# jrkerns/pylinac

Measured on NVIDIA H100. Metric: EPID frames/sec (1024x1024) through PicketFence.analyze(), higher is better.
Workload: dtype u16 pixels / int exact sums / f64 profiles

## Files before the change

pylinac_b200/csrc/peaks.cuh:

```cuda
#pragma once
#include "common.cuh"

namespace epid {

constexpr int PK_WALK = 64;
#ifndef EPID_PK_MAXBLK
#define EPID_PK_MAXBLK 512
#endif
constexpr int PK_MAXBLK = EPID_PK_MAXBLK;
constexpr int PK_RANK_MAX = 768;
constexpr int PK_COOP = 32;

struct PeakArgs {
    double hmin;
    int distance;
    double pmin;
    double wmin;
    double rel_height;
    int max_number;
    int sort_by_height;
};

struct PeakWork {
    int cap;
    int* idx;
    double* prom;
    int* lbase;
    int* rbase;
    double* width_height;
    double* lip;
    double* rip;
    int* flag;
    double* skey;
    int* sidx;
    int* s_small;
};

__device__ __forceinline__ bool key_less(double ka, int ia, double kb, int ib) { return ka < kb || (ka == kb && ia < ib); }

__device__ inline void block_bitonic_sort(double* key, int* idx, int m) {
    for (int k = 2; k <= m; k <<= 1) {
        for (int j = k >> 1; j > 0; j >>= 1) {
            for (int i = threadIdx.x; i < m; i += blockDim.x) {
                const int l = i ^ j;
                if (l > i) {
                    const bool up = (i & k) == 0;
                    const double ka = key[i], kb = key[l];
                    const int ia = idx[i], ib = idx[l];
                    const bool sw = up ? key_less(kb, ib, ka, ia) : key_less(ka, ia, kb, ib);
                    if (sw) {
                        key[i] = kb; key[l] = ka;
                        idx[i] = ib; idx[l] = ia;
                    }
                }
            }
            __syncthreads();
        }
    }
}

__device__ inline int compact_by_flag(PeakWork& w, int count, bool have_props) {
    const int tid = threadIdx.x, nt = blockDim.x, lane = tid & 31, wid = tid >> 5, nw = nt >> 5;
    __syncthreads();
    int out = 0;
    for (int base = 0; base < count; base += nt) {
        const int i = base + tid;
        const bool keep = i < count && w.flag[i] != 0;
        int idx = 0, lb = 0, rb = 0;
// ... 94 lines not shown
            bool waiting = false;
            for (int i = tid; i < count; i += nt) {
                int st = cur[i];
                if (st == 2) {
                    const int pi = w.idx[i], ri = rank[i];
                    bool has_kept = false, blocked = false;
                    for (int k = i - 1; k >= 0 && pi - w.idx[k] < a.distance; k--) {
                        const int sk = cur[k];
                        if (sk == 1) { has_kept = true; break; }
                        if (sk == 2 && rank[k] > ri) { blocked = true; break; }
                    }
                    if (!has_kept && !blocked) {
                        for (int k = i + 1; k < count && w.idx[k] - pi < a.distance; k++) {
                            const int sk = cur[k];
                            if (sk == 1) { has_kept = true; break; }
                            if (sk == 2 && rank[k] > ri) { blocked = true; break; }
                        }
                    }
                    st = has_kept ? 0 : (blocked ? 2 : 1);
                    waiting = waiting || st == 2;
                }
                nxt[i] = st;
            }
            const int more = __syncthreads_or(waiting ? 1 : 0);
            int* t = cur; cur = nxt; nxt = t;
            if (!more) break;
        }
        if (cur != w.flag) {
            for (int i = tid; i < count; i += nt) w.flag[i] = cur[i];
        }
        count = compact_by_flag(w, count, false);
    }

    __shared__ double s_bmax[PK_MAXBLK], s_bmin[PK_MAXBLK];
    __shared__ unsigned short s_bpos[PK_MAXBLK];
    const bool have_tab = n <= 32 * PK_MAXBLK;
    if (have_tab) {
        const int lane = tid & 31, wid = tid >> 5, nw = nt >> 5;
        const int nblk = (n + 31) >> 5;
        __syncthreads();
        for (int b = wid; b < nblk; b += nw) {
            const int k = (b << 5) + lane;
            const bool in = k < n;
            const double v = in ? x[k] : 0.0;
            double vmax = in ? v : -__longlong_as_double(0x7ff0000000000000LL);
            double vmin = in ? v : __longlong_as_double(0x7ff0000000000000LL);
#pragma unroll
            for (int o = 16; o > 0; o >>= 1) {
                vmax = fmax(vmax, __shfl_xor_sync(0xffffffffu, vmax, o));
                vmin = fmin(vmin, __shfl_xor_sync(0xffffffffu, vmin, o));
            }
            const unsigned eq = __ballot_sync(0xffffffffu, in && v == vmin);
            if (lane == 0) {
                s_bmax[b] = vmax;
                s_bmin[b] = vmin;
                s_bpos[b] = (unsigned short)((__ffs(eq) - 1) | ((31 - __clz(eq)) << 8));
            }
        }
        __syncthreads();
        for (int i = tid; i < count; i += nt) {
            const int p = w.idx[i];
            const double xp = x[p];
            const int pb_ = p >> 5;
            double lmin = xp;
            int lb = p;
            bool stop = false;
            for (int k = p; k >= (pb_ << 5); k--) {
                const double v = x[k];
                if (!stop) {
                    if (v > xp) stop = true;
                    else if (v < lmin) { lmin = v; lb = k; }
                }
            }
            for (int b = pb_ - 1; b >= 0 && !stop; b--) {
                if (s_bmax[b] > xp) {
                    for (int k = (b << 5) + 31; k >= (b << 5); k--) {
                        const double v = x[k];
                        if (!stop) {
                            if (v > xp) stop = true;
                            else if (v < lmin) { lmin = v; lb = k; }
                        }
                    }
                } else if (s_bmin[b] < lmin) {
                    lmin = s_bmin[b];
                    lb = (b << 5) + (s_bpos[b] >> 8);
                }
            }
            double rmin = xp;
            int rb = p;
            stop = false;
            const int own_end = min(n - 1, (pb_ << 5) + 31);
            for (int k = p; k <= own_end; k++) {
// ... 187 lines not shown
```

pylinac_b200/csrc/pf_common.cuh:

```cuda
#pragma once
#include <cmath>

#include "filters.cuh"
#include "peaks.cuh"
#include "stats.cuh"

namespace epid {

constexpr int PF_P = EPID_PF_MAX_PICKETS;
constexpr int PF_L = EPID_PF_MAX_LEAVES;
constexpr int PROF_THREADS = 256;
constexpr int PROF_MAXN = STATS_MAX_DIM;
constexpr int PROF_PEAK_CAP = 512;
constexpr int WIN_WARPS = 4;
constexpr int WIN_CAP_PX = 4096;
constexpr int WIN_MAX_NC = 1024;
constexpr int WIN_MAX_NR = 64;
constexpr int FIN_THREADS = 256;

constexpr int PF_STATUS_DEFERRED = 90;

struct PfConst {
    epid_pf_params p;
    int H, W;
// ... 187 lines not shown
    const int wid = threadIdx.x >> 5, nw = blockDim.x >> 5, lane = threadIdx.x & 31;
    __syncthreads();
    if (n0 <= 1024 && n1 <= 1024) {
        for (int s = wid; s < 4; s += nw) {
            const bool second = s >= 2;
            const PctPlan& pp = (s & 1) ? (second ? p99_1 : p99_0) : (second ? p85_1 : p85_0);
            uint32_t va, vb;
            warp_select_pair_u32(second ? a1 : a0, second ? n1 : n0, pp.prev, pp.next, va, vb);
            if (lane == 0) { sel[2 * s] = va; sel[2 * s + 1] = vb; }
        }
    } else {
        for (int s = wid; s < 8; s += nw) {
            const bool second = s >= 4;
            const PctPlan& pp = (s & 2) ? (second ? p99_1 : p99_0) : (second ? p85_1 : p85_0);
            const int r = (s & 1) ? pp.next : pp.prev;
            const uint32_t v = warp_select_u32(second ? a1 : a0, second ? n1 : n0, r);
            if (lane == 0) sel[s] = v;
        }
    }
    __syncthreads();
    range0 = np_lerp((double)sel[2], (double)sel[3], p99_0.gamma) - np_lerp((double)sel[0], (double)sel[1], p85_0.gamma);
    range1 = np_lerp((double)sel[6], (double)sel[7], p99_1.gamma) - np_lerp((double)sel[4], (double)sel[5], p85_1.gamma);
    __syncthreads();
}

__host__ __device__ inline int pf_profile_len(int H, int W) { return ((H > W ? H : W) + 3) & ~3; }
__host__ __device__ inline size_t pf_profile_smem_bytes(int threads, int H, int W) {
    return sizeof(double) * (pf_profile_len(H, W) + 5 * PROF_PEAK_CAP) + sizeof(int) * (5 * PROF_PEAK_CAP + threads + 8) + 64 * sizeof(double);
}

__device__ inline void pf_profile_block(const PfConst& c, PfFrame& f, const uint32_t* __restrict__ rowsum,
                                        const uint32_t* __restrict__ colsum, const uint32_t* __restrict__ rowsum2,
                                        const uint32_t* __restrict__ colsum2, unsigned char* smraw, double d_colsum2 = 0.0,
                                        double d_rowsum2 = 0.0, int* counters = nullptr) {
    double* prof = reinterpret_cast<double*>(smraw);
    double* w_prom = prof + pf_profile_len(c.H, c.W);
    double* w_wh = w_prom + PROF_PEAK_CAP;
    double* w_lip = w_wh + PROF_PEAK_CAP;
    double* w_rip = w_lip + PROF_PEAK_CAP;
    double* w_skey = w_rip + PROF_PEAK_CAP;
    double* s_red = w_skey + PROF_PEAK_CAP;
    double* s_bcast = s_red + 32;
    int* w_idx = reinterpret_cast<int*>(s_bcast + 32);
    int* w_lb = w_idx + PROF_PEAK_CAP;
    int* w_rb = w_lb + PROF_PEAK_CAP;
    int* w_flag = w_rb + PROF_PEAK_CAP;
    int* w_sidx = w_flag + PROF_PEAK_CAP;
    int* w_small = w_sidx + PROF_PEAK_CAP;

    if (f.status != EPID_PF_OK) return;
    const int H = c.H, W = c.W;
    const int tid = threadIdx.x;
    const int NT = blockDim.x;
    const int NW = NT >> 5;

    int orient = c.p.orientation;
    if (orient < 0) {
        uint32_t* buf = reinterpret_cast<uint32_t*>(prof);
        double row_range, col_range;
        block_pct_ranges2(colsum2, W, c.p85[0], c.p99[0], rowsum2, H, c.p85[1], c.p99[1], buf, row_range, col_range);
        orient = (row_range < col_range) ? 1 : 0;
        if (counters && (d_colsum2 > 0.0 || d_rowsum2 > 0.0)) {
            const bool sure_lr = row_range + d_colsum2 + 1.0 < col_range - d_rowsum2;
            const bool sure_ud = row_range - d_colsum2 >= col_range + d_rowsum2 + 1.0;
            if (!sure_lr && !sure_ud) {
                if (threadIdx.x == 0) { atomicAdd(&counters[1], 1); f.status = PF_STATUS_DEFERRED; }
                return;
            }
        }
    }
    const int n = orient == 0 ? W : H;
    const int other = orient == 0 ? H : W;
    const uint32_t* raw = orient == 0 ? colsum : rowsum;
    const long long base = (long long)other * (long long)(f.inv ? f.mx : f.mn);
    double lmax = 0.0;
    for (int i = tid; i < n; i += NT) {
        const long long sg = f.inv ? base - (long long)raw[i] : (long long)raw[i] - base;
        const double v = (double)sg;
        prof[i] = v;
        lmax = fmax(lmax, v);
    }
    lmax = warp_max(lmax);
    if ((tid & 31) == 0) s_red[tid >> 5] = lmax;
    __syncthreads();
    if (tid == 0) {
        double m = 0.0;
        for (int i = 0; i < NW; i++) m = fmax(m, s_red[i]);
        s_bcast[0] = m;
    }
    __syncthreads();
    const double pmax = s_bcast[0];
    double lmin = 2.0;
    for (int i = tid; i < n; i += NT) {
        const double v = prof[i] / pmax;
        prof[i] = v;
        lmin = fmin(lmin, v);
    }
    lmin = warp_min(lmin);
    __syncthreads();
    if ((tid & 31) == 0) s_red[tid >> 5] = lmin;
    __syncthreads();
    if (tid == 0) {
        double m = 2.0;
        for (int i = 0; i < NW; i++) m = fmin(m, s_red[i]);
        s_bcast[1] = m;
    }
    __syncthreads();
    const double pmin = s_bcast[1];
    PeakArgs a;
    {
        const double val_range = 1.0 - pmin;
        double thr = c.p.height_threshold;
        if (thr >= 0.0 && thr <= 1.0) thr = pmin + thr * val_range;
        a.hmin = thr;
        a.distance = max((int)(0.02 * (double)n), 1);
        a.pmin = c.p.required_prominence;
        a.wmin = 0.0;
        a.rel_height = 1.0 - 0.5;
        a.max_number = c.p.num_pickets;
        a.sort_by_height = c.p.peak_sort == 1;
    }
    PeakWork w;
    w.cap = PROF_PEAK_CAP;
    w.idx = w_idx; w.prom = w_prom; w.lbase = w_lb; w.rbase = w_rb; w.width_height = w_wh; w.lip = w_lip; w.rip = w_rip;
    w.flag = w_flag; w.skey = w_skey; w.sidx = w_sidx; w.s_small = w_small;
    const int np = block_find_peaks(prof, n, a, w);
    if (tid == 0) {
        f.orientation = orient;
        if (np < 0 || np > PF_P) {
            f.status = EPID_PF_TOO_MANY_PICKETS;
        } else if (np == 0) {
            f.status = EPID_PF_NO_PICKETS;
        } else {
            f.n_pickets = np;
            int sorted[PF_P];
            for (int k = 0; k < np; k++) {
                const double lt = w.lip[k], rt = w.rip[k];
                const int idx = (int)rint(lt + (rt - lt) / 2.0);
                f.picket_idx[k] = idx;
                f.picket_val[k] = prof[idx];
                int j = k;
                while (j > 0 && sorted[j - 1] > idx) { sorted[j] = sorted[j - 1]; j--; }
                sorted[j] = idx;
            }
            double spacing = c.p.picket_spacing;
            if (spacing < 0) {
                const int nd = np - 1;
                if (nd <= 0) {
                    spacing = __longlong_as_double(0x7ff8000000000000LL);
                } else {
                    int d[PF_P];
                    for (int k = 0; k < nd; k++) {
                        const int v = sorted[k + 1] - sorted[k];
                        int j = k;
                        while (j > 0 && d[j - 1] > v) { d[j] = d[j - 1]; j--; }
                        d[j] = v;
                    }
                    spacing = (nd & 1) ? (double)d[nd / 2] : ((double)d[nd / 2 - 1] + (double)d[nd / 2]) / 2.0;
                }
            }
            f.spacing = spacing;
            if (spacing != spacing) f.status = EPID_PF_NAN_SPACING;
            const double n_axis = (double)(orient == 0 ? H : W);
            const double ratio = c.p.leaf_analysis_width_ratio;
            double pixel_range = n_axis / 2.0;
            pixel_range -= fmax(c.p.leaf_width_mm[0] * ratio, c.p.leaf_width_mm[c.p.n_leaves - 1] * ratio) * c.p.dpmm;
            int cnt = 0;
            for (int l = 0; l < c.p.n_leaves; l++)
                if (fabs(c.p.leaf_center_mm[l]) < pixel_range / c.p.dpmm) f.inview[cnt++] = (short)l;
            f.n_inview = cnt;
        }
    }
}

}
```

pylinac_b200/csrc/pf_stream.cu:

```cuda
#define EPID_PK_MAXBLK 2
#include "pf_common.cuh"
#include "tma.cuh"

namespace epid {

#ifndef EPID_ST_NCW
#define EPID_ST_NCW 12
#endif
constexpr int ST_NCW = EPID_ST_NCW;
constexpr int ST_THREADS = (ST_NCW + 1) * 32;
constexpr int ST_NST = 6;
constexpr int ST_KMAX = 8;
constexpr int ST_MAXROWS = 1024;
constexpr int PILOT_THREADS = 256;
constexpr int PILOT_BINS = 2048;
constexpr int PILOT_STEP = 32, PILOT_OFF = 16;
constexpr int TAIL_THREADS = 256;

struct PilotOut {
    uint32_t u_lo, a1, b1, l_hi;
};

struct ItemOut {
    uint32_t mn, mx;
    uint32_t cnt_a, cnt_b, cnt_lo, cnt_hi;
    uint32_t pad[2];
};

struct StreamGeom {
    int H, W;
    int K;
    int rows_per_item;
    int nvec;
    int nstrips;
    int wa;
    int row_bytes;
    int rps;
};

__device__ __forceinline__ void consumer_bar() { asm volatile("bar.sync 1, %0;" ::"n"(ST_NCW * 32) : "memory"); }
__device__ __forceinline__ uint4 lds128(uint32_t addr) {
    uint4 r;
    asm volatile("ld.shared.v4.u32 {%0,%1,%2,%3}, [%4];" : "=r"(r.x), "=r"(r.y), "=r"(r.z), "=r"(r.w) : "r"(addr));
    return r;
}

__device__ __forceinline__ int pilot_rows_of(int H) { return H > PILOT_OFF ? (H - PILOT_OFF + PILOT_STEP - 1) / PILOT_STEP : 0; }

__device__ __forceinline__ uint32_t pilot_scan_excl(uint32_t v, uint32_t* s_red, uint32_t* total) {
    const int lane = threadIdx.x & 31, wid = threadIdx.x >> 5;
    uint32_t inc = v;
#pragma unroll
    for (int o = 1; o < 32; o <<= 1) {
        const uint32_t t = __shfl_up_sync(0xffffffffu, inc, o);
        if (lane >= o) inc += t;
    }
    __syncthreads();
    if (lane == 31) s_red[wid] = inc;
    __syncthreads();
    if (wid == 0) {
        const uint32_t w = lane < PILOT_THREADS / 32 ? s_red[lane] : 0;
        uint32_t winc = w;
#pragma unroll
        for (int o = 1; o < 32; o <<= 1) {
            const uint32_t t = __shfl_up_sync(0xffffffffu, winc, o);
            if (lane >= o) winc += t;
        }
        if (lane < PILOT_THREADS / 32) s_red[lane] = winc - w;
        if (lane == 31) s_red[32] = winc;
    }
    __syncthreads();
    const uint32_t excl = s_red[wid] + inc - v;
    *total = s_red[32];
    return excl;
}

__device__ inline uint32_t pilot_find(const uint32_t* __restrict__ hist, uint32_t nb, uint32_t base, uint32_t rank, uint32_t* s_red,
                                      uint32_t* s_found) {
    const int tid = threadIdx.x;
    const uint32_t per = (nb + PILOT_THREADS - 1) / PILOT_THREADS;
    const uint32_t lo = min(nb, tid * per), hi = min(nb, lo + per);
    uint32_t c = 0;
    for (uint32_t i = lo; i < hi; i++) c += hist[i];
    uint32_t total;
    const uint32_t excl = pilot_scan_excl(c, s_red, &total);
    if (tid == 0) *s_found = rank < base ? 0xffffffffu : nb;
    __syncthreads();
    if (rank >= base) {
        const uint32_t k = rank - base;
        if (k >= excl && k < excl + c) {
            uint32_t acc = excl;
            for (uint32_t i = lo; i < hi; i++) {
                const uint32_t h = hist[i];
                if (k < acc + h) { *s_found = i; break; }
                acc += h;
            }
        }
    }
    __syncthreads();
    const uint32_t r = *s_found;
    __syncthreads();
    return r;
}

__global__ void __launch_bounds__(PILOT_THREADS)
k_pf_pilot(const StatsGeom g, const FrameRef* __restrict__ frames, int nframes, PilotOut* __restrict__ out) {
    __shared__ uint32_t hist[3][PILOT_BINS];
    __shared__ uint32_t bis_lo[4], bis_hi[4], bis_cnt[4], bis_rank[4];
    __shared__ uint32_t a0s[3], b0s[3], shs[3], below_s[3], eq_s[3];
    __shared__ uint32_t s_red[40], s_found, smin, smax;
    const int fi = blockIdx.x;
    if (fi >= nframes) return;
    const FrameRef frf = frames[fi];
    const int H = g.H, W = g.W;
    const int tid = threadIdx.x, lane = tid & 31, wid = tid >> 5;
    const uint32_t npix = (uint32_t)H * (uint32_t)W;
    const uint32_t k_lo[3] = {g.ranks[0], g.ranks[4], npix - 1 - g.ranks[3]};
    const uint32_t k_hi[3] = {g.ranks[1], g.ranks[5], npix - 1 - g.ranks[2]};
    for (int i = tid; i < 3 * PILOT_BINS; i += PILOT_THREADS) (&hist[0][0])[i] = 0;
    if (tid < 3) { below_s[tid] = 0; eq_s[tid] = 0; }
    if (tid == 0) { smin = 0xffffu; smax = 0; }
    uint32_t sv[8];
    {
        const int col = min(W - 1, (int)(((long long)tid * W) / PILOT_THREADS));
#pragma unroll
        for (int i = 0; i < 8; i++) {
            const int row = min(H - 1, (int)(((2 * i + 1) * (long long)H) / 16));
            sv[i] = __ldg(frf.origin + (size_t)row * frf.pitch + col);
        }
    }
    const uint32_t nT0 = PILOT_THREADS * 8;
    if (tid < 4) {
        const int b = tid == 0 ? 0 : (tid == 3 ? 2 : 1);
        const double fq = fmin((b == 1 ? 1.0 : 4.0) * (double)(tid == 1 ? k_lo[b] : k_hi[b]) / (double)npix, 0.999);
        const double sg = sqrt(fq * (1.0 - fq) * (double)nT0);
        const double ctr = fq * (double)nT0;
        double rr = (tid == 1) ? ctr - 5.0 * sg - 2.0 : ctr + 5.0 * sg + 3.0;
        rr = fmin(fmax(rr, 0.0), (double)(nT0 - 1));
        bis_rank[tid] = (uint32_t)rr;
        bis_lo[tid] = 0;
        bis_hi[tid] = 65535u;
        bis_cnt[tid] = 0;
    }
    __syncthreads();
    {
        uint32_t mnv = sv[0], mxv = sv[0];
#pragma unroll
        for (int i = 1; i < 8; i++) { mnv = min(mnv, sv[i]); mxv = max(mxv, sv[i]); }
        mnv = warp_min(mnv);
        mxv = warp_max(mxv);
        if (lane == 0) { atomicMin(&smin, mnv); atomicMax(&smax, mxv); }
    }
    for (int step = 0; step < 16; step++) {
        uint32_t cnt[4];
#pragma unroll
        for (int t = 0; t < 4; t++) {
            const uint32_t mid = (bis_lo[t] + bis_hi[t]) >> 1;
            uint32_t cc_ = 0;
#pragma unroll
            for (int i = 0; i < 8; i++) {
                const uint32_t v = t == 3 ? 65535u - sv[i] : sv[i];
                cc_ += v <= mid ? 1u : 0u;
            }
            cnt[t] = __reduce_add_sync(0xffffffffu, cc_);
        }
        if (lane < 4) atomicAdd(&bis_cnt[lane], lane == 0 ? cnt[0] : lane == 1 ? cnt[1] : lane == 2 ? cnt[2] : cnt[3]);
        __syncthreads();
        if (tid < 4) {
            const uint32_t mid = (bis_lo[tid] + bis_hi[tid]) >> 1;
            if (bis_cnt[tid] >= bis_rank[tid] + 1) bis_hi[tid] = mid; else bis_lo[tid] = mid + 1;
            bis_cnt[tid] = 0;
        }
        __syncthreads();
    }
    if (tid == 0) {
        uint32_t a[3], b[3];
        a[0] = smin;              b[0] = max(bis_lo[0], smin);
        a[1] = bis_lo[1];         b[1] = max(bis_lo[2], a[1]);
        a[2] = 65535u - smax;     b[2] = max(bis_lo[3], a[2]);
        for (int j = 0; j < 3; j++) {
            uint32_t sh = 0;
            while (((b[j] - a[j]) >> sh) >= (uint32_t)PILOT_BINS) sh++;
            a0s[j] = a[j];
            b0s[j] = b[j];
            shs[j] = sh;
        }
    }
    __syncthreads();
    const uint32_t a0[3] = {a0s[0], a0s[1], a0s[2]};
    const uint32_t wd[3] = {b0s[0] - a0s[0], b0s[1] - a0s[1], b0s[2] - a0s[2]};
    const uint32_t sh[3] = {shs[0], shs[1], shs[2]};
    uint32_t below[3] = {0, 0, 0}, eq[3] = {0, 0, 0};
    const int np_rows = pilot_rows_of(H);
    const bool aligned = true;
    const int mis = (int)((reinterpret_cast<uintptr_t>(frf.origin) >> 1) & 7);
    const int jf = (mis + 7) / 8, jl = (W + mis) / 8;
    const int cl = aligned ? min(W, max(0, jf * 8 - mis)) : 0;
    const int cr = aligned ? (jl > jf ? jl * 8 - mis : cl) : 0;
    auto put = [&](int j, uint32_t vv) {
        const int u = (int)vv - (int)a0[j];
        below[j] += (uint32_t)u >> 31;
        eq[j] += u == 0 ? 1u : 0u;
        if ((uint32_t)(u - 1) < wd[j]) atomicAdd(&hist[j][(uint32_t)u >> sh[j]], 1u);
    };
    for (int ri = wid; ri < np_rows; ri += PILOT_THREADS / 32) {
        const uint16_t* rowp = frf.origin + (size_t)(PILOT_OFF + PILOT_STEP * ri) * frf.pitch;
        for (int j = jf + lane; j < jl; j += 32) {
            const uint4 q = ldg_stream16(rowp - mis + j * 8);
            const uint32_t w[4] = {q.x, q.y, q.z, q.w};
            const uint32_t vm = __vminu2(__vminu2(w[0], w[1]), __vminu2(w[2], w[3]));
            const uint32_t vM = __vmaxu2(__vmaxu2(w[0], w[1]), __vmaxu2(w[2], w[3]));
            put(0, vm & 0xffffu);
            put(0, vm >> 16);
            put(2, 65535u - (vM & 0xffffu));
            put(2, 65535u - (vM >> 16));
#pragma unroll
            for (int t = 0; t < 4; t++) { put(1, w[t] & 0xffffu); put(1, w[t] >> 16); }
        }
    }
#pragma unroll
    for (int j = 0; j < 3; j++) {
        const uint32_t b = __reduce_add_sync(0xffffffffu, below[j]);
        const uint32_t e = __reduce_add_sync(0xffffffffu, eq[j]);
        if (lane == 0) { if (b) atomicAdd(&below_s[j], b); if (e) atomicAdd(&eq_s[j], e); }
    }
    __syncthreads();
    if (tid < 3 && eq_s[tid]) hist[tid][0] += eq_s[tid];
    __syncthreads();
    const uint32_t n_p = (uint32_t)np_rows * (uint32_t)(aligned ? cr - cl : W);
    uint32_t thr_lo[3], thr_hi[3];
    for (int j = 0; j < 3; j++) {
        const uint32_t nb = (wd[j] >> sh[j]) + 1;
        const double scale = (double)n_p / (double)npix;
        const double pop = j == 1 ? (double)n_p : (double)n_p / 4.0;
        const double fq = fmin((j == 1 ? 1.0 : 4.0) * ((double)k_lo[j] + 0.5) / (double)npix, 1.0);
        const double sg = sqrt(fq * (1.0 - fq) * pop);
        const double rl = (double)k_lo[j] * scale - 5.0 * sg - 2.0;
        const double ru = (double)k_hi[j] * scale + 5.0 * sg + 3.0;
        const uint32_t r_l = rl <= 0.0 ? 0u : (uint32_t)rl;
        const uint32_t r_u = (uint32_t)fmin(ru, fmax(pop - 1.0, 0.0));
        const uint32_t xa = pilot_find(hist[j], nb, below_s[j], r_l, s_red, &s_found);
        const uint32_t xb = pilot_find(hist[j], nb, below_s[j], r_u, s_red, &s_found);
        uint32_t lo_t = xa == 0xffffffffu ? a0[j] : a0[j] + (min(xa, nb - 1) << sh[j]);
        uint32_t hi_t = xb == 0xffffffffu ? a0[j] : a0[j] + (((min(xb, nb - 1) + 1) << sh[j]) - 1);
        hi_t = min(hi_t, 65535u);
        lo_t = min(lo_t, hi_t);
        thr_lo[j] = lo_t;
        thr_hi[j] = hi_t;
    }
    if (tid == 0) {
        PilotOut o;
        o.u_lo = thr_hi[0];
        o.a1 = thr_lo[1];
        o.b1 = thr_hi[1];
        o.l_hi = 65535u - thr_hi[2];
        out[fi] = o;
    }
}

struct StreamSh {
    unsigned long long full[ST_NST], empty[ST_NST];
    uint32_t mn, mx, cnt[4];
};

template <int VPL>
__global__ void __launch_bounds__(ST_THREADS, 1)
k_pf_stream(const StreamGeom sg, const FrameRef* __restrict__ frames, const PilotOut* __restrict__ pilot, int nitems,
            ItemOut* __restrict__ items, uint32_t* __restrict__ col_raw, uint32_t* __restrict__ col_cl,
            uint32_t* __restrict__ row_raw, uint32_t* __restrict__ row_cl) {
    extern __shared__ __align__(128) unsigned char smraw[];
    StreamSh* sh = reinterpret_cast<StreamSh*>(smraw);
    unsigned char* ring = smraw + 256;
    const int stage_bytes = sg.rps * sg.row_bytes;
    uint32_t* flush = reinterpret_cast<uint32_t*>(ring + (size_t)ST_NST * stage_bytes);
    const int tid = threadIdx.x, lane = tid & 31, wid = tid >> 5;
    if (tid == 0) {
        for (int s = 0; s < ST_NST; s++) { mbar_init(smem_u32(&sh->full[s]), 1); mbar_init(smem_u32(&sh->empty[s]), ST_NCW); }
// ... 155 lines not shown
          const uint32_t* __restrict__ col_cl, const uint32_t* __restrict__ row_raw, const uint32_t* __restrict__ row_cl,
          PfFrame* fr, FrameStats* __restrict__ stats, int* counters) {
    extern __shared__ __align__(128) unsigned char smraw[];
    __shared__ uint32_t s_mn, s_mx, s_cnt[4], s_flag;
    __shared__ unsigned long long s_sum, s_corner;
    const PfConst& c = *cc;
    const int fi = blockIdx.x;
    const int H = g.H, W = g.W;
    const int Hp = (H + 3) & ~3, Wp = (W + 3) & ~3;
    uint32_t* rowsum_sm = reinterpret_cast<uint32_t*>(smraw);
    uint32_t* colsum_sm = rowsum_sm + Hp;
    uint32_t* rowsum2_sm = colsum_sm + Wp;
    uint32_t* colsum2_sm = rowsum2_sm + Hp;
    unsigned char* prof_raw = reinterpret_cast<unsigned char*>(colsum2_sm + Wp);
    const int tid = threadIdx.x, lane = tid & 31;
    PfFrame& f = fr[fi];
    const FrameRef frf = frames[fi];
    const PilotOut po = pilot[fi];
    const int mis = (int)((reinterpret_cast<uintptr_t>(frf.origin) >> 1) & 7);
    const uint32_t npix = (uint32_t)H * (uint32_t)W;
    if (tid == 0) { s_mn = 0xffffu; s_mx = 0; s_cnt[0] = s_cnt[1] = s_cnt[2] = s_cnt[3] = 0; s_sum = 0; s_corner = 0; s_flag = 0; }
    for (int x = tid; x < W; x += TAIL_THREADS) {
        const int ac = x + mis;
        uint32_t a = 0, b = 0;
        if (ac < sg.wa) {
            for (int k = 0; k < sg.K; k++) {
                a += col_raw[((size_t)fi * sg.K + k) * sg.wa + ac];
                b += col_cl[((size_t)fi * sg.K + k) * sg.wa + ac];
            }
        }
        colsum_sm[x] = a;
        colsum2_sm[x] = b;
    }
    for (int y = tid; y < H; y += TAIL_THREADS) {
        uint32_t a = 0, b = 0;
        for (int s = 0; s < sg.nstrips; s++) {
            a += row_raw[((size_t)fi * 2 + s) * H + y];
            b += row_cl[((size_t)fi * 2 + s) * H + y];
        }
        rowsum_sm[y] = a;
        rowsum2_sm[y] = b;
    }
    __syncthreads();
    if (tid < sg.K) {
        const ItemOut o = items[(size_t)fi * sg.K + tid];
        atomicMin(&s_mn, o.mn);
        atomicMax(&s_mx, o.mx);
        atomicAdd(&s_cnt[0], o.cnt_a);
        atomicAdd(&s_cnt[1], o.cnt_b);
        atomicAdd(&s_cnt[2], o.cnt_lo);
        atomicAdd(&s_cnt[3], o.cnt_hi);
    }
    {
        const int jf = (mis + 7) / 8, jl = (W + mis) / 8;
        const int cl = min(W, max(0, jf * 8 - mis)), cr = jl > jf ? jl * 8 - mis : cl;
        const int ne = cl + (W - cr);
        uint32_t mnv = 0xffffu, mxv = 0, e0 = 0, e1 = 0, e2 = 0, e3 = 0;
        for (int i = tid; i < ne * H; i += TAIL_THREADS) {
            const int r = i / ne, e = i - r * ne;
            const int cidx = e < cl ? e : cr + (e - cl);
            const uint32_t v = __ldg(frf.origin + (size_t)r * frf.pitch + cidx);
            const uint32_t xa = max(v, po.a1);
            mnv = min(mnv, v);
            mxv = max(mxv, v);
            atomicAdd(&rowsum_sm[r], v);
            atomicAdd(&colsum_sm[cidx], v);
            atomicAdd(&rowsum2_sm[r], xa);
            atomicAdd(&colsum2_sm[cidx], xa);
            e0 += v < po.a1 ? 1u : 0u;
            e1 += v <= po.b1 ? 1u : 0u;
            e2 += v <= po.u_lo ? 1u : 0u;
            e3 += v >= po.l_hi ? 1u : 0u;
        }
        if (ne > 0) {
            mnv = warp_min(mnv); mxv = warp_max(mxv);
            e0 = warp_sum(e0); e1 = warp_sum(e1); e2 = warp_sum(e2); e3 = warp_sum(e3);
            if (lane == 0) {
                atomicMin(&s_mn, mnv); atomicMax(&s_mx, mxv);
                atomicAdd(&s_cnt[0], e0); atomicAdd(&s_cnt[1], e1); atomicAdd(&s_cnt[2], e2); atomicAdd(&s_cnt[3], e3);
            }
        }
    }
    if (g.box > 0) {
        const int per = g.box * g.box;
        unsigned long long cs = 0;
        for (int i = tid; i < 4 * per; i += TAIL_THREADS) {
            const int b = i / per, o = i - b * per;
            const int y = o / g.box, x = o - y * g.box;
            const int rr = ((b & 2) ? H - g.rp - g.box : g.rp) + y;
            const int cl = ((b & 1) ? W - g.cp - g.box : g.cp) + x;
            if (rr >= 0 && rr < H && cl >= 0 && cl < W) cs += __ldg(frf.origin + (size_t)rr * frf.pitch + cl);
        }
        cs = warp_sum(cs);
        if (lane == 0 && cs) atomicAdd(&s_corner, cs);
    }
    __syncthreads();
    {
        unsigned long long tsum = 0;
        for (int i = tid; i < H; i += TAIL_THREADS) tsum += rowsum_sm[i];
        tsum = warp_sum(tsum);
        if (lane == 0) atomicAdd(&s_sum, tsum);
    }
    __syncthreads();
    if (tid == 0) {
        const uint32_t mn = s_mn, mx = s_mx;
        f.status = EPID_PF_OK;
        f.noisy = 0;
        f.noise_passes = 0;
        f.n_pickets = 0;
        f.n_inview = 0;
        f.todo = 0;
        f.win2 = 0;
        f.orientation = 0;
        f.mn = mn;
        f.mx = mx;
        f.D = mx - mn;
        int bad = 0;
        if (f.D == 0) {
            f.status = EPID_PF_FLAT_IMAGE;
            f.inv = 0;
            f.corner_inverted = 0;
            f.med2 = 0;
        } else {
            const double avg = (double)s_corner / (double)(4 * 10 * 10);
            const double mean = (double)s_sum / (double)npix;
            f.corner_inverted = avg > mean ? 1 : 0;
            f.inv = f.corner_inverted ^ (c.p.invert ? 1 : 0);
            const uint32_t cnt_a = s_cnt[0];
            const uint32_t cnt_b = po.b1 >= 65535u ? npix : s_cnt[1];
            const uint32_t cnt_lo = po.u_lo >= 65535u ? npix : s_cnt[2];
            const uint32_t cnt_hi = po.l_hi == 0u ? npix : s_cnt[3];
            if (!(cnt_a <= g.ranks[4] && cnt_b >= g.ranks[5] + 1u)) bad = 1;
            if (!(cnt_lo >= g.ranks[1] + 1u && cnt_hi >= npix - g.ranks[2])) bad = 1;
            const double near_min = (double)min(po.u_lo, mx), near_max = (double)max(po.l_hi, mn);
            const double mnv = (double)mn, mxv = (double)mx;
            const bool max_is_extreme = mxv > near_max * 1.25;
            const bool min_is_extreme = (mnv < near_min * 0.75) && (fabs(mnv - near_min) > 0.1 * (near_max - near_min));
            if (max_is_extreme || min_is_extreme) bad = 1;
            f.med2 = f.inv ? 2u * (mx - min(po.a1, mx)) : 2u * (max(po.a1, mn) - mn);
        }
        FrameStats st;
        st.mn = mn; st.mx = mx; st.npix = npix; st.inv_certified = 0;
        st.sum = s_sum; st.corner_sum = s_corner;
        for (int i = 0; i < STATS_MAX_RANKS; i++) st.ostat[i] = 0;
        st.ostat[0] = mn; st.ostat[1] = po.u_lo; st.ostat[2] = po.l_hi; st.ostat[3] = mx; st.ostat[4] = po.a1; st.ostat[5] = po.b1;
        stats[fi] = st;
        if (bad) { atomicAdd(&counters[1], 1); s_flag = 1; f.status = PF_STATUS_DEFERRED; }
    }
    __syncthreads();
    if (s_flag || f.status != EPID_PF_OK) return;
    double d_row = 0.0, d_col = 0.0;
    if (c.p.orientation < 0) {
        const uint32_t mn = f.mn, mx = f.mx, a1 = po.a1;
        const int inv = f.inv;
        for (int y = tid; y < H; y += TAIL_THREADS) {
            const uint32_t raw = rowsum_sm[y], cl = rowsum2_sm[y];
            rowsum2_sm[y] = !inv ? 2u * cl - 2u * mn * (uint32_t)W : 2u * mx * (uint32_t)W - 2u * (raw + a1 * (uint32_t)W - cl);
        }
        for (int x = tid; x < W; x += TAIL_THREADS) {
            const uint32_t raw = colsum_sm[x], cl = colsum2_sm[x];
            colsum2_sm[x] = !inv ? 2u * cl - 2u * mn * (uint32_t)H : 2u * mx * (uint32_t)H - 2u * (raw + a1 * (uint32_t)H - cl);
        }
        d_row = 2.0 * (double)(po.b1 - po.a1) * (double)W;
        d_col = 2.0 * (double)(po.b1 - po.a1) * (double)H;
    }
    __syncthreads();
    pf_profile_block(c, f, rowsum_sm, colsum_sm, rowsum2_sm, colsum2_sm, prof_raw, d_col, d_row, counters);
}

size_t pf_tail_smem_bytes(int H, int W) {
    const int Hp = (H + 3) & ~3, Wp = (W + 3) & ~3;
    return sizeof(uint32_t) * (size_t)(2 * Hp + 2 * Wp) + pf_profile_smem_bytes(TAIL_THREADS, H, W) + 64;
}

static int stream_vpl(int nvec, int* nstrips) {
    int ns = nvec <= 128 ? 1 : 2;
    int vpl = (nvec + 32 * ns - 1) / (32 * ns);
    *nstrips = ns;
    return vpl;
}

bool pf_front_supported(int H, int W, int pitch) {
    if ((pitch % 8) != 0 || H < 64 || W < 64 || H > STATS_MAX_DIM || W > STATS_MAX_DIM) return false;
    int ns;
    const int nvec = (W + 7 + 7) / 8;
    const int vpl = stream_vpl(nvec, &ns);
    if (vpl > 4) return false;
    if ((H + ST_KMAX - 1) / ST_KMAX > ST_MAXROWS) return false;
    return pf_tail_smem_bytes(H, W) <= 200 * 1024;
}

size_t pf_front_scratch_bytes(int n, int H, int W) {
    return 256 * 8 + sizeof(PilotOut) * (size_t)n + sizeof(ItemOut) * (size_t)n * ST_KMAX +
           2 * sizeof(uint32_t) * (size_t)n * ST_KMAX * 2048 + 2 * sizeof(uint32_t) * (size_t)n * 2 * H;
}

template <int VPL>
static int launch_stream(epid_ctx* ctx, cudaStream_t stream, int grid, size_t smem, const StreamGeom& sg, const FrameRef* refs, const PilotOut* pilot,
                         int nitems, ItemOut* items, uint32_t* col_raw, uint32_t* col_cl, uint32_t* row_raw, uint32_t* row_cl) {
    EPID_SMEM_OPT_IN(ctx, k_pf_stream<VPL>, smem);
// ... 60 lines not shown
```

Measured before the change: 472,100.

## Restructure pilot quantile search, tail reductions, and peak prominence walk

The pilot kernel now runs all six rank searches over the three histograms in one pass with a single set of barriers instead of separate scan/find calls, and it software-pipelines its row loads with a 4-deep uint4 prefetch and occupancy launch bounds. The tail kernel folds the total sum into the row and remainder loops, merges the profile max/min reductions to cut barriers, and finalises pickets (sorting, median spacing, in-view leaves) with one warp of shuffles instead of a single thread. The peak prominence walk gets a warp-per-peak path for small peak counts and reuses the caller's rowsum buffer as its block min/max table, re-enabling the table that was previously shrunk to two entries. Several compile-time skip macros for profiling are also added.

```diff
diff --git a/pylinac_b200/csrc/peaks.cuh b/pylinac_b200/csrc/peaks.cuh
--- a/pylinac_b200/csrc/peaks.cuh
+++ b/pylinac_b200/csrc/peaks.cuh
@@ -34,6 +34,10 @@
     double* skey;
     int* sidx;
     int* s_small;
+    double* tab_max = nullptr;
+    double* tab_min = nullptr;
+    unsigned short* tab_pos = nullptr;
+    int tab_blk = 0;
 };
 
 __device__ __forceinline__ bool key_less(double ka, int ia, double kb, int ib) { return ka < kb || (ka == kb && ia < ib); }
@@ -194,9 +198,16 @@
         count = compact_by_flag(w, count, false);
     }
 
+#ifdef EPID_PK_CALLER_TABLE
+    double* s_bmax = w.tab_max;
+    double* s_bmin = w.tab_min;
+    unsigned short* s_bpos = w.tab_pos;
+    constexpr bool have_tab = true;
+#else
     __shared__ double s_bmax[PK_MAXBLK], s_bmin[PK_MAXBLK];
     __shared__ unsigned short s_bpos[PK_MAXBLK];
     const bool have_tab = n <= 32 * PK_MAXBLK;
+#endif
     if (have_tab) {
         const int lane = tid & 31, wid = tid >> 5, nw = nt >> 5;
         const int nblk = (n + 31) >> 5;
@@ -220,6 +231,43 @@
             }
         }
         __syncthreads();
+        if (count <= 4 * nw) {
+            const double inf = __longlong_as_double(0x7ff0000000000000LL);
+            for (int i = wid; i < count; i += nw) {
+                const int p = w.idx[i];
+                const double xp = x[p];
+                double lmin = inf, rmin = inf;
+                int lb = p, rb = p;
+                for (int k0 = p;; k0 -= 32) {
+                    const int k = k0 - lane;
+                    const double v = k >= 0 ? x[k] : 0.0;
+                    const unsigned stop = __ballot_sync(0xffffffffu, k >= 0 && v > xp);
+                    const int lim = stop ? __ffs(stop) - 1 : 32;
+                    if (lane < lim && k >= 0 && v < lmin) { lmin = v; lb = k; }
+                    if (stop || k0 < 32) break;
+                }
+                for (int k0 = p;; k0 += 32) {
+                    const int k = k0 + lane;
+                    const double v = k < n ? x[k] : 0.0;
+                    const unsigned stop = __ballot_sync(0xffffffffu, k < n && v > xp);
+                    const int lim = stop ? __ffs(stop) - 1 : 32;
+                    if (lane < lim && k < n && v < rmin) { rmin = v; rb = k; }
+                    if (stop || k0 + 32 >= n) break;
+                }
+#pragma unroll
+                for (int o = 16; o > 0; o >>= 1) {
+                    const double ol = __shfl_xor_sync(0xffffffffu, lmin, o), orr = __shfl_xor_sync(0xffffffffu, rmin, o);
+                    const int olb = __shfl_xor_sync(0xffffffffu, lb, o), orb = __shfl_xor_sync(0xffffffffu, rb, o);
+                    if (ol < lmin || (ol == lmin && olb > lb)) { lmin = ol; lb = olb; }
+                    if (orr < rmin || (orr == rmin && orb < rb)) { rmin = orr; rb = orb; }
+                }
+                if (lane == 0) {
+                    w.prom[i] = xp - fmax(lmin, rmin);
+                    w.lbase[i] = lb;
+                    w.rbase[i] = rb;
+                }
+            }
+        } else
         for (int i = tid; i < count; i += nt) {
             const int p = w.idx[i];
             const double xp = x[p];
diff --git a/pylinac_b200/csrc/pf_common.cuh b/pylinac_b200/csrc/pf_common.cuh
--- a/pylinac_b200/csrc/pf_common.cuh
+++ b/pylinac_b200/csrc/pf_common.cuh
@@ -243,7 +243,7 @@
 __device__ inline void pf_profile_block(const PfConst& c, PfFrame& f, const uint32_t* __restrict__ rowsum,
                                         const uint32_t* __restrict__ colsum, const uint32_t* __restrict__ rowsum2,
                                         const uint32_t* __restrict__ colsum2, unsigned char* smraw, double d_colsum2 = 0.0,
-                                        double d_rowsum2 = 0.0, int* counters = nullptr) {
+                                        double d_rowsum2 = 0.0, int* counters = nullptr, unsigned char* peak_tab = nullptr) {
     double* prof = reinterpret_cast<double*>(smraw);
     double* w_prom = prof + pf_profile_len(c.H, c.W);
     double* w_wh = w_prom + PROF_PEAK_CAP;
@@ -284,40 +284,23 @@
     const int other = orient == 0 ? H : W;
     const uint32_t* raw = orient == 0 ? colsum : rowsum;
     const long long base = (long long)other * (long long)(f.inv ? f.mx : f.mn);
-    double lmax = 0.0;
+    double lmax = 0.0, lmin = __longlong_as_double(0x7ff0000000000000LL);
     for (int i = tid; i < n; i += NT) {
         const long long sg = f.inv ? base - (long long)raw[i] : (long long)raw[i] - base;
         const double v = (double)sg;
         prof[i] = v;
         lmax = fmax(lmax, v);
+        lmin = fmin(lmin, v);
     }
     lmax = warp_max(lmax);
-    if ((tid & 31) == 0) s_red[tid >> 5] = lmax;
+    lmin = warp_min(lmin);
+    if ((tid & 31) == 0) { s_red[tid >> 5] = lmax; s_bcast[tid >> 5] = lmin; }
     __syncthreads();
-    if (tid == 0) {
-        double m = 0.0;
-        for (int i = 0; i < NW; i++) m = fmax(m, s_red[i]);
-        s_bcast[0] = m;
-    }
+    double pmax = 0.0, rmin = s_bcast[0];
+    for (int i = 0; i < NW; i++) { pmax = fmax(pmax, s_red[i]); rmin = fmin(rmin, s_bcast[i]); }
+    for (int i = tid; i < n; i += NT) prof[i] = prof[i] / pmax;
+    const double pmin = rmin / pmax;
     __syncthreads();
-    const double pmax = s_bcast[0];
-    double lmin = 2.0;
-    for (int i = tid; i < n; i += NT) {
-        const double v = prof[i] / pmax;
-        prof[i] = v;
-        lmin = fmin(lmin, v);
-    }
-    lmin = warp_min(lmin);
-    __syncthreads();
-    if ((tid & 31) == 0) s_red[tid >> 5] = lmin;
-    __syncthreads();
-    if (tid == 0) {
-        double m = 2.0;
-        for (int i = 0; i < NW; i++) m = fmin(m, s_red[i]);
-        s_bcast[1] = m;
-    }
-    __syncthreads();
-    const double pmin = s_bcast[1];
     PeakArgs a;
     {
         const double val_range = 1.0 - pmin;
@@ -335,24 +318,43 @@
     w.cap = PROF_PEAK_CAP;
     w.idx = w_idx; w.prom = w_prom; w.lbase = w_lb; w.rbase = w_rb; w.width_height = w_wh; w.lip = w_lip; w.rip = w_rip;
     w.flag = w_flag; w.skey = w_skey; w.sidx = w_sidx; w.s_small = w_small;
+    if (peak_tab) {
+        w.tab_blk = (n + 31) >> 5;
+        w.tab_max = reinterpret_cast<double*>(peak_tab);
+        w.tab_min = w.tab_max + w.tab_blk;
+        w.tab_pos = reinterpret_cast<unsigned short*>(w.tab_min + w.tab_blk);
+    }
+#ifdef EPID_TAIL_SKIP_PEAKS
+    const int np = 0;
+#else
     const int np = block_find_peaks(prof, n, a, w);
-    if (tid == 0) {
-        f.orientation = orient;
+#endif
+    static_assert(PF_P <= 32, "one lane per picket");
+    if (tid < 32) {
+        const int lane = tid;
+        if (lane == 0) f.orientation = orient;
         if (np < 0 || np > PF_P) {
-            f.status = EPID_PF_TOO_MANY_PICKETS;
+            if (lane == 0) f.status = EPID_PF_TOO_MANY_PICKETS;
         } else if (np == 0) {
-            f.status = EPID_PF_NO_PICKETS;
+            if (lane == 0) f.status = EPID_PF_NO_PICKETS;
         } else {
-            f.n_pickets = np;
-            int sorted[PF_P];
-            for (int k = 0; k < np; k++) {
-                const double lt = w.lip[k], rt = w.rip[k];
-                const int idx = (int)rint(lt + (rt - lt) / 2.0);
-                f.picket_idx[k] = idx;
-                f.picket_val[k] = prof[idx];
-                int j = k;
-                while (j > 0 && sorted[j - 1] > idx) { sorted[j] = sorted[j - 1]; j--; }
-                sorted[j] = idx;
+            const bool mine = lane < np;
+            int idx = 0x7fffffff;
+            if (mine) {
+                const double lt = w.lip[lane], rt = w.rip[lane];
+                idx = (int)rint(lt + (rt - lt) / 2.0);
+                f.picket_idx[lane] = idx;
+                f.picket_val[lane] = prof[idx];
+            }
+            int rank = 0;
+            for (int j = 0; j < 32; j++) {
+                const int o = __shfl_sync(0xffffffffu, idx, j);
+                rank += (o < idx || (o == idx && j < lane)) ? 1 : 0;
+            }
+            int sorted = 0;
+            for (int j = 0; j < 32; j++) {
+                const int o = __shfl_sync(0xffffffffu, idx, j), r = __shfl_sync(0xffffffffu, rank, j);
+                if (r == lane) sorted = o;
             }
             double spacing = c.p.picket_spacing;
             if (spacing < 0) {
@@ -360,28 +362,40 @@
                 if (nd <= 0) {
                     spacing = __longlong_as_double(0x7ff8000000000000LL);
                 } else {
-                    int d[PF_P];
-                    for (int k = 0; k < nd; k++) {
-                        const int v = sorted[k + 1] - sorted[k];
-                        int j = k;
-                        while (j > 0 && d[j - 1] > v) { d[j] = d[j - 1]; j--; }
-                        d[j] = v;
+                    const int nxt = __shfl_down_sync(0xffffffffu, sorted, 1);
+                    const int d = lane < nd ? nxt - sorted : 0x7fffffff;
+                    int drank = 0;
+                    for (int j = 0; j < 32; j++) {
+                        const int o = __shfl_sync(0xffffffffu, d, j);
+                        drank += (o < d || (o == d && j < lane)) ? 1 : 0;
                     }
-                    spacing = (nd & 1) ? (double)d[nd / 2] : ((double)d[nd / 2 - 1] + (double)d[nd / 2]) / 2.0;
+                    const unsigned hi = __ballot_sync(0xffffffffu, lane < nd && drank == nd / 2);
+                    const unsigned lo = __ballot_sync(0xffffffffu, lane < nd && drank == nd / 2 - 1);
+                    const int d_hi = __shfl_sync(0xffffffffu, d, __ffs(hi) - 1);
+                    const int d_lo = __shfl_sync(0xffffffffu, d, lo ? __ffs(lo) - 1 : 0);
+                    spacing = (nd & 1) ? (double)d_hi : ((double)d_lo + (double)d_hi) / 2.0;
                 }
             }
-            f.spacing = spacing;
-            if (spacing != spacing) f.status = EPID_PF_NAN_SPACING;
+            if (lane == 0) {
+                f.n_pickets = np;
+                f.spacing = spacing;
+                if (spacing != spacing) f.status = EPID_PF_NAN_SPACING;
+            }
             const double n_axis = (double)(orient == 0 ? H : W);
             const double ratio = c.p.leaf_analysis_width_ratio;
             double pixel_range = n_axis / 2.0;
             pixel_range -= fmax(c.p.leaf_width_mm[0] * ratio, c.p.leaf_width_mm[c.p.n_leaves - 1] * ratio) * c.p.dpmm;
             int cnt = 0;
-            for (int l = 0; l < c.p.n_leaves; l++)
-                if (fabs(c.p.leaf_center_mm[l]) < pixel_range / c.p.dpmm) f.inview[cnt++] = (short)l;
-            f.n_inview = cnt;
-        }
-    }
-}
-
-}
+            for (int l0 = 0; l0 < c.p.n_leaves; l0 += 32) {
+                const int l = l0 + lane;
+                const bool in = l < c.p.n_leaves && fabs(c.p.leaf_center_mm[l]) < pixel_range / c.p.dpmm;
+                const unsigned b = __ballot_sync(0xffffffffu, in);
+                if (in) f.inview[cnt + __popc(b & ((1u << lane) - 1u))] = (short)l;
+                cnt += __popc(b);
+            }
+            if (lane == 0) f.n_inview = cnt;
+        }
+    }
+}
+
+}
diff --git a/pylinac_b200/csrc/pf_stream.cu b/pylinac_b200/csrc/pf_stream.cu
--- a/pylinac_b200/csrc/pf_stream.cu
+++ b/pylinac_b200/csrc/pf_stream.cu
@@ -1,4 +1,4 @@
-#define EPID_PK_MAXBLK 2
+#define EPID_PK_CALLER_TABLE
 #include "pf_common.cuh"
 #include "tma.cuh"
 
@@ -47,80 +47,100 @@
 
 __device__ __forceinline__ int pilot_rows_of(int H) { return H > PILOT_OFF ? (H - PILOT_OFF + PILOT_STEP - 1) / PILOT_STEP : 0; }
 
-__device__ __forceinline__ uint32_t pilot_scan_excl(uint32_t v, uint32_t* s_red, uint32_t* total) {
-    const int lane = threadIdx.x & 31, wid = threadIdx.x >> 5;
-    uint32_t inc = v;
-#pragma unroll
-    for (int o = 1; o < 32; o <<= 1) {
-        const uint32_t t = __shfl_up_sync(0xffffffffu, inc, o);
-        if (lane >= o) inc += t;
-    }
-    __syncthreads();
-    if (lane == 31) s_red[wid] = inc;
-    __syncthreads();
-    if (wid == 0) {
-        const uint32_t w = lane < PILOT_THREADS / 32 ? s_red[lane] : 0;
-        uint32_t winc = w;
+constexpr int PILOT_WARPS = PILOT_THREADS / 32;
+
+__device__ __forceinline__ void pilot_find_all(const uint32_t (*__restrict__ hist)[PILOT_BINS], const uint32_t nb[3], const uint32_t base[3],
+                                      const uint32_t rk[3][2], uint32_t* s_red, uint32_t* s_found, uint32_t xs[3][2]) {
+    const int tid = threadIdx.x, lane = tid & 31, wid = tid >> 5;
+    auto chunk = [&](int j, uint32_t& lo, uint32_t& hi) {
+        const uint32_t per = (nb[j] + PILOT_THREADS - 1) / PILOT_THREADS;
+        lo = min(nb[j], tid * per);
+        hi = min(nb[j], lo + per);
+    };
+    uint32_t c[3], inc[3];
+#pragma unroll
+    for (int j = 0; j < 3; j++) {
+        uint32_t lo, hi;
+        chunk(j, lo, hi);
+        c[j] = 0;
+        for (uint32_t i = lo; i < hi; i++) c[j] += hist[j][i];
+        inc[j] = c[j];
 #pragma unroll
         for (int o = 1; o < 32; o <<= 1) {
-            const uint32_t t = __shfl_up_sync(0xffffffffu, winc, o);
-            if (lane >= o) winc += t;
-        }
-        if (lane < PILOT_THREADS / 32) s_red[lane] = winc - w;
-        if (lane == 31) s_red[32] = winc;
-    }
-    __syncthreads();
-    const uint32_t excl = s_red[wid] + inc - v;
-    *total = s_red[32];
-    return excl;
-}
-
-__device__ inline uint32_t pilot_find(const uint32_t* __restrict__ hist, uint32_t nb, uint32_t base, uint32_t rank, uint32_t* s_red,
-                                      uint32_t* s_found) {
-    const int tid = threadIdx.x;
-    const uint32_t per = (nb + PILOT_THREADS - 1) / PILOT_THREADS;
-    const uint32_t lo = min(nb, tid * per), hi = min(nb, lo + per);
-    uint32_t c = 0;
-    for (uint32_t i = lo; i < hi; i++) c += hist[i];
-    uint32_t total;
-    const uint32_t excl = pilot_scan_excl(c, s_red, &total);
-    if (tid == 0) *s_found = rank < base ? 0xffffffffu : nb;
-    __syncthreads();
-    if (rank >= base) {
-        const uint32_t k = rank - base;
-        if (k >= excl && k < excl + c) {
-            uint32_t acc = excl;
-            for (uint32_t i = lo; i < hi; i++) {
-                const uint32_t h = hist[i];
-                if (k < acc + h) { *s_found = i; break; }
-                acc += h;
-            }
-        }
-    }
-    __syncthreads();
-    const uint32_t r = *s_found;
-    __syncthreads();
-    return r;
-}
-
-__global__ void __launch_bounds__(PILOT_THREADS)
+            const uint32_t t = __shfl_up_sync(0xffffffffu, inc[j], o);
+            if (lane >= o) inc[j] += t;
+        }
+        if (lane == 31) s_red[j * PILOT_WARPS + wid] = inc[j];
+    }
+#pragma unroll
+    for (int q = 0; q < 6; q++)
+        if (tid == q) s_found[q] = rk[q >> 1][q & 1] < base[q >> 1] ? 0xffffffffu : nb[q >> 1];
+    __syncthreads();
+#pragma unroll
+    for (int j = 0; j < 3; j++) {
+        uint32_t excl = inc[j] - c[j];
+        for (int w = 0; w < wid; w++) excl += s_red[j * PILOT_WARPS + w];
+#pragma unroll
+        for (int k = 0; k < 2; k++) {
+            if (rk[j][k] < base[j]) continue;
+            const uint32_t kk = rk[j][k] - base[j];
+            if (kk >= excl && kk < excl + c[j]) {
+                uint32_t lo, hi, acc = excl;
+                chunk(j, lo, hi);
+                for (uint32_t i = lo; i < hi; i++) {
+                    const uint32_t h = hist[j][i];
+                    if (kk < acc + h) { s_found[2 * j + k] = i; break; }
+                    acc += h;
+                }
+            }
+        }
+    }
+    __syncthreads();
+#pragma unroll
+    for (int j = 0; j < 3; j++) { xs[j][0] = s_found[2 * j]; xs[j][1] = s_found[2 * j + 1]; }
+}
+
+__global__ void __launch_bounds__(PILOT_THREADS, 4)
 k_pf_pilot(const StatsGeom g, const FrameRef* __restrict__ frames, int nframes, PilotOut* __restrict__ out) {
     __shared__ uint32_t hist[3][PILOT_BINS];
     __shared__ uint32_t bis_lo[4], bis_hi[4], bis_cnt[4], bis_rank[4];
-    __shared__ uint32_t a0s[3], b0s[3], shs[3], below_s[3], eq_s[3];
-    __shared__ uint32_t s_red[40], s_found, smin, smax;
+    __shared__ uint32_t below_s[3], eq_s[3];
+    __shared__ uint32_t s_red[3 * PILOT_WARPS], s_found[6], smin, smax;
     const int fi = blockIdx.x;
     if (fi >= nframes) return;
     const FrameRef frf = frames[fi];
     const int H = g.H, W = g.W;
     const int tid = threadIdx.x, lane = tid & 31, wid = tid >> 5;
     const uint32_t npix = (uint32_t)H * (uint32_t)W;
-    const uint32_t k_lo[3] = {g.ranks[0], g.ranks[4], npix - 1 - g.ranks[3]};
-    const uint32_t k_hi[3] = {g.ranks[1], g.ranks[5], npix - 1 - g.ranks[2]};
+    const int np_rows = pilot_rows_of(H);
+    const int mis = (int)((reinterpret_cast<uintptr_t>(frf.origin) >> 1) & 7);
+    const int jf = (mis + 7) / 8, jl = (W + mis) / 8;
+    const int cl = min(W, max(0, jf * 8 - mis));
+    const int cr = jl > jf ? jl * 8 - mis : cl;
+#ifdef EPID_PILOT_SKIP_ROWS
+    const int ntask = 0;
+#else
+    const int ntask = (wid < np_rows ? (np_rows - 1 - wid) / PILOT_WARPS + 1 : 0) * ((jl - jf + 127) / 128);
+#endif
+    const uint16_t* t_row = frf.origin - mis + (size_t)(PILOT_OFF + PILOT_STEP * wid) * frf.pitch;
+    int t_j0 = jf + lane, qn_j0 = 0;
+    auto load_next = [&](uint4 (&q)[4]) {
+        qn_j0 = t_j0;
+#pragma unroll
+        for (int u = 0; u < 4; u++) {
+            const int j = t_j0 + 32 * u;
+            q[u] = j < jl ? ldg_stream16(t_row + j * 8) : make_uint4(0, 0, 0, 0);
+        }
+        t_j0 += 128;
+        if (t_j0 >= jl) { t_j0 = jf + lane; t_row += (size_t)(PILOT_STEP * PILOT_WARPS) * frf.pitch; }
+    };
+    auto k_lo = [&](int j) { return j == 0 ? g.ranks[0] : j == 1 ? g.ranks[4] : npix - 1 - g.ranks[3]; };
+    auto k_hi = [&](int j) { return j == 0 ? g.ranks[1] : j == 1 ? g.ranks[5] : npix - 1 - g.ranks[2]; };
     for (int i = tid; i < 3 * PILOT_BINS; i += PILOT_THREADS) (&hist[0][0])[i] = 0;
     if (tid < 3) { below_s[tid] = 0; eq_s[tid] = 0; }
     if (tid == 0) { smin = 0xffffu; smax = 0; }
     uint32_t sv[8];
+#ifndef EPID_PILOT_SKIP_T0
     {
         const int col = min(W - 1, (int)(((long long)tid * W) / PILOT_THREADS));
 #pragma unroll
@@ -129,10 +149,11 @@
             sv[i] = __ldg(frf.origin + (size_t)row * frf.pitch + col);
         }
     }
+#endif
     const uint32_t nT0 = PILOT_THREADS * 8;
     if (tid < 4) {
         const int b = tid == 0 ? 0 : (tid == 3 ? 2 : 1);
-        const double fq = fmin((b == 1 ? 1.0 : 4.0) * (double)(tid == 1 ? k_lo[b] : k_hi[b]) / (double)npix, 0.999);
+        const double fq = fmin((b == 1 ? 1.0 : 4.0) * (double)(tid == 1 ? k_lo(b) : k_hi(b)) / (double)npix, 0.999);
         const double sg = sqrt(fq * (1.0 - fq) * (double)nT0);
         const double ctr = fq * (double)nT0;
         double rr = (tid == 1) ? ctr - 5.0 * sg - 2.0 : ctr + 5.0 * sg + 3.0;
@@ -143,6 +164,10 @@
         bis_cnt[tid] = 0;
     }
     __syncthreads();
+#ifdef EPID_PILOT_SKIP_T0
+    if (tid == 0) { smin = 0; smax = 65535u; bis_lo[0] = bis_lo[2] = bis_lo[3] = 65535u; bis_lo[1] = 0; }
+    __syncthreads();
+#else
     {
         uint32_t mnv = sv[0], mxv = sv[0];
 #pragma unroll
@@ -173,41 +198,40 @@
         }
         __syncthreads();
     }
-    if (tid == 0) {
-        uint32_t a[3], b[3];
-        a[0] = smin;              b[0] = max(bis_lo[0], smin);
-        a[1] = bis_lo[1];         b[1] = max(bis_lo[2], a[1]);
-        a[2] = 65535u - smax;     b[2] = max(bis_lo[3], a[2]);
+#endif
+    uint4 qn[4];
+    if (ntask > 0) load_next(qn);
+    uint32_t a0[3], wd[3], sh[3];
+    {
+        const uint32_t s_mn = smin, s_mx = smax;
+        uint32_t b[3];
+        a0[0] = s_mn;             b[0] = max(bis_lo[0], s_mn);
+        a0[1] = bis_lo[1];        b[1] = max(bis_lo[2], a0[1]);
+        a0[2] = 65535u - s_mx;    b[2] = max(bis_lo[3], a0[2]);
+#pragma unroll
         for (int j = 0; j < 3; j++) {
-            uint32_t sh = 0;
-            while (((b[j] - a[j]) >> sh) >= (uint32_t)PILOT_BINS) sh++;
-            a0s[j] = a[j];
-            b0s[j] = b[j];
-            shs[j] = sh;
-        }
-    }
-    __syncthreads();
-    const uint32_t a0[3] = {a0s[0], a0s[1], a0s[2]};
-    const uint32_t wd[3] = {b0s[0] - a0s[0], b0s[1] - a0s[1], b0s[2] - a0s[2]};
-    const uint32_t sh[3] = {shs[0], shs[1], shs[2]};
+            wd[j] = b[j] - a0[j];
+            sh[j] = 0;
+            while ((wd[j] >> sh[j]) >= (uint32_t)PILOT_BINS) sh[j]++;
+        }
+    }
     uint32_t below[3] = {0, 0, 0}, eq[3] = {0, 0, 0};
-    const int np_rows = pilot_rows_of(H);
-    const bool aligned = true;
-    const int mis = (int)((reinterpret_cast<uintptr_t>(frf.origin) >> 1) & 7);
-    const int jf = (mis + 7) / 8, jl = (W + mis) / 8;
-    const int cl = aligned ? min(W, max(0, jf * 8 - mis)) : 0;
-    const int cr = aligned ? (jl > jf ? jl * 8 - mis : cl) : 0;
     auto put = [&](int j, uint32_t vv) {
         const int u = (int)vv - (int)a0[j];
         below[j] += (uint32_t)u >> 31;
         eq[j] += u == 0 ? 1u : 0u;
         if ((uint32_t)(u - 1) < wd[j]) atomicAdd(&hist[j][(uint32_t)u >> sh[j]], 1u);
     };
-    for (int ri = wid; ri < np_rows; ri += PILOT_THREADS / 32) {
-        const uint16_t* rowp = frf.origin + (size_t)(PILOT_OFF + PILOT_STEP * ri) * frf.pitch;
-        for (int j = jf + lane; j < jl; j += 32) {
-            const uint4 q = ldg_stream16(rowp - mis + j * 8);
-            const uint32_t w[4] = {q.x, q.y, q.z, q.w};
+    for (int t = 0; t < ntask; t++) {
+        uint4 q[4];
+#pragma unroll
+        for (int u = 0; u < 4; u++) q[u] = qn[u];
+        const int j0 = qn_j0;
+        if (t + 1 < ntask) load_next(qn);
+#pragma unroll
+        for (int u = 0; u < 4; u++) {
+            if (j0 + 32 * u >= jl) continue;
+            const uint32_t w[4] = {q[u].x, q[u].y, q[u].z, q[u].w};
             const uint32_t vm = __vminu2(__vminu2(w[0], w[1]), __vminu2(w[2], w[3]));
             const uint32_t vM = __vmaxu2(__vmaxu2(w[0], w[1]), __vmaxu2(w[2], w[3]));
             put(0, vm & 0xffffu);
@@ -215,7 +239,7 @@
             put(2, 65535u - (vM & 0xffffu));
             put(2, 65535u - (vM >> 16));
 #pragma unroll
-            for (int t = 0; t < 4; t++) { put(1, w[t] & 0xffffu); put(1, w[t] >> 16); }
+            for (int k = 0; k < 4; k++) { put(1, w[k] & 0xffffu); put(1, w[k] >> 16); }
         }
     }
 #pragma unroll
@@ -227,22 +251,33 @@
     __syncthreads();
     if (tid < 3 && eq_s[tid]) hist[tid][0] += eq_s[tid];
     __syncthreads();
-    const uint32_t n_p = (uint32_t)np_rows * (uint32_t)(aligned ? cr - cl : W);
-    uint32_t thr_lo[3], thr_hi[3];
+    const uint32_t n_p = (uint32_t)np_rows * (uint32_t)(cr - cl);
+    uint32_t nb[3], base[3], rk[3][2];
+#pragma unroll
     for (int j = 0; j < 3; j++) {
-        const uint32_t nb = (wd[j] >> sh[j]) + 1;
+        nb[j] = (wd[j] >> sh[j]) + 1;
+        base[j] = below_s[j];
         const double scale = (double)n_p / (double)npix;
         const double pop = j == 1 ? (double)n_p : (double)n_p / 4.0;
-        const double fq = fmin((j == 1 ? 1.0 : 4.0) * ((double)k_lo[j] + 0.5) / (double)npix, 1.0);
+        const double fq = fmin((j == 1 ? 1.0 : 4.0) * ((double)k_lo(j) + 0.5) / (double)npix, 1.0);
         const double sg = sqrt(fq * (1.0 - fq) * pop);
-        const double rl = (double)k_lo[j] * scale - 5.0 * sg - 2.0;
-        const double ru = (double)k_hi[j] * scale + 5.0 * sg + 3.0;
-        const uint32_t r_l = rl <= 0.0 ? 0u : (uint32_t)rl;
-        const uint32_t r_u = (uint32_t)fmin(ru, fmax(pop - 1.0, 0.0));
-        const uint32_t xa = pilot_find(hist[j], nb, below_s[j], r_l, s_red, &s_found);
-        const uint32_t xb = pilot_find(hist[j], nb, below_s[j], r_u, s_red, &s_found);
-        uint32_t lo_t = xa == 0xffffffffu ? a0[j] : a0[j] + (min(xa, nb - 1) << sh[j]);
-        uint32_t hi_t = xb == 0xffffffffu ? a0[j] : a0[j] + (((min(xb, nb - 1) + 1) << sh[j]) - 1);
+        const double rl = (double)k_lo(j) * scale - 5.0 * sg - 2.0;
+        const double ru = (double)k_hi(j) * scale + 5.0 * sg + 3.0;
+        rk[j][0] = rl <= 0.0 ? 0u : (uint32_t)rl;
+        rk[j][1] = (uint32_t)fmin(ru, fmax(pop - 1.0, 0.0));
+    }
+    uint32_t xs[3][2];
+#ifdef EPID_PILOT_SKIP_FIND
+    for (int j = 0; j < 3; j++) xs[j][0] = xs[j][1] = 0;
+#else
+    pilot_find_all(hist, nb, base, rk, s_red, s_found, xs);
+#endif
+    uint32_t thr_lo[3], thr_hi[3];
+#pragma unroll
+    for (int j = 0; j < 3; j++) {
+        const uint32_t xa = xs[j][0], xb = xs[j][1];
+        uint32_t lo_t = xa == 0xffffffffu ? a0[j] : a0[j] + (min(xa, nb[j] - 1) << sh[j]);
+        uint32_t hi_t = xb == 0xffffffffu ? a0[j] : a0[j] + (((min(xb, nb[j] - 1) + 1) << sh[j]) - 1);
         hi_t = min(hi_t, 65535u);
         lo_t = min(lo_t, hi_t);
         thr_lo[j] = lo_t;
@@ -464,6 +499,7 @@
         colsum_sm[x] = a;
         colsum2_sm[x] = b;
     }
+    unsigned long long tsum = 0;
     for (int y = tid; y < H; y += TAIL_THREADS) {
         uint32_t a = 0, b = 0;
         for (int s = 0; s < sg.nstrips; s++) {
@@ -472,6 +508,7 @@
         }
         rowsum_sm[y] = a;
         rowsum2_sm[y] = b;
+        tsum += a;
     }
     __syncthreads();
     if (tid < sg.K) {
@@ -499,6 +536,7 @@
             atomicAdd(&colsum_sm[cidx], v);
             atomicAdd(&rowsum2_sm[r], xa);
             atomicAdd(&colsum2_sm[cidx], xa);
+            tsum += v;
             e0 += v < po.a1 ? 1u : 0u;
             e1 += v <= po.b1 ? 1u : 0u;
             e2 += v <= po.u_lo ? 1u : 0u;
@@ -526,13 +564,8 @@
         cs = warp_sum(cs);
         if (lane == 0 && cs) atomicAdd(&s_corner, cs);
     }
-    __syncthreads();
-    {
-        unsigned long long tsum = 0;
-        for (int i = tid; i < H; i += TAIL_THREADS) tsum += rowsum_sm[i];
-        tsum = warp_sum(tsum);
-        if (lane == 0) atomicAdd(&s_sum, tsum);
-    }
+    tsum = warp_sum(tsum);
+    if (lane == 0) atomicAdd(&s_sum, tsum);
     __syncthreads();
     if (tid == 0) {
         const uint32_t mn = s_mn, mx = s_mx;
@@ -597,7 +630,11 @@
         d_col = 2.0 * (double)(po.b1 - po.a1) * (double)H;
     }
     __syncthreads();
-    pf_profile_block(c, f, rowsum_sm, colsum_sm, rowsum2_sm, colsum2_sm, prof_raw, d_col, d_row, counters);
+#ifdef EPID_TAIL_SKIP_PROFILE
+    return;
+#endif
+    pf_profile_block(c, f, rowsum_sm, colsum_sm, rowsum2_sm, colsum2_sm, prof_raw, d_col, d_row, counters,
+                     reinterpret_cast<unsigned char*>(rowsum_sm));
 }
 
 size_t pf_tail_smem_bytes(int H, int W) {
```

After: 490,600, median of 6. 3.9% higher.
